# Xinglab/lr2rmats

Measured on AMD Instinct MI355X. Metric: long-read alignments classified/sec; achieved HBM GB/s vs roofline, higher is better.
Workload: dtype int32

## Files before the change

### lr2rmats_amd/csrc/l2r_engine.hip

```cpp
#include <hip/hip_runtime.h>
#include <stdarg.h>
#include <stdio.h>
#include <stdlib.h>
#include <string.h>
#include <sys/stat.h>
#include <unistd.h>
#include <algorithm>
#include <string>
#include <thread>
#include <type_traits>
#include <utility>
#include <vector>

#include "../../include/lr2rmats_hip.h"
#include "l2r_kernels.hip.h"
#include "l2r_window.hip.h"
#include "l2r_slab.hip.h"
#include "l2r_chunk.hip.h"
#include "l2r_tchunk.hip.h"
#include "l2r_filter.hip.h"
#include "l2r_fusion.hip.h"
#include "l2r_sj.hip.h"
#include "l2r_plan.hip.h"

// ... 70 lines not shown
    ~SjState() { for (int k = 0; k < 2; ++k) if (ev[k]) (void)hipEventDestroy(ev[k]); }
};
struct SjIntrons {
    DevBuf<int32_t> tx_tid, ex_start, ex_end; DevBuf<int64_t> tx_ex_off;
    SjState st;
};

struct RunFacts {
    bool known = false;
    uint32_t n_wide = 0;
    uint32_t n_chunk = 0;
    uint32_t n_rest = 0;
    uint32_t n_late = 0;
    uint32_t n_fb = 0;
    uint32_t n_wide_rest = 0;
    unsigned long long chunk_rest = 0;
    bool redo_empty = false;
};

struct l2r_ctx {
    int device = 0;
    hipStream_t stream = nullptr;
    hipStream_t side[2] = {nullptr, nullptr};
    hipEvent_t ev_fork = nullptr, ev_join[2] = {nullptr, nullptr};

    int fast_grid = 0;
    int n_cu = 256, wg_per_cu = 4;
    int ablate = 0;
    int64_t seg_max = SEG_MAX;
    Pipeline want_pipe = Pipeline::tile;
    bool pipeline_forced = false;
    bool wide_direct = true;
    bool chunk_direct = true;
    bool tile_split = true;
    bool side_on = true;
    bool env_tile_anyway = false, env_launch_all = false;
    bool check_stages = false;
    bool env_stamps = false;
    int64_t tile_resident = 0;
    bool tile_starved = false;
    int64_t n_lb_fallback = 0;

    l2r_params prm;
    std::string anno_cache_dir;
    int anno_cache_state = 0;
    unsigned want = L2R_WANT_RESULTS | L2R_WANT_ACCEPTED;
    bool one_shot_upload = false;

    bool sorted = true;
    int reads_per_tile = TILE_THREADS;
    int64_t n_tiles = 0, n_tiles256 = 0;
    bool wide_cigar = false;
    bool many_exon_reads = false;
    bool slab_ok = false;
    bool have_index = false;
    float index_ms = 0.0f;
    DevBuf<SlotRec> slot_rec;
    DevBuf<TileStat> tile_stat; std::vector<TileStat> h_tile_stat;
    DevBuf<TileStat> sup_stat;
    DevBuf<uint16_t> sum_nn;
    DevBuf<uint32_t> tile_sbase, s_pre, s_loc, s_pl, cig_off32, tile_rec, tile_total, tile_xbase, tile_span;
    DevBuf<int32_t> dense_start, dense_end;
    DevBuf<uint32_t> slab_row;
    DevBuf<TileWin> tw;
    DevBuf<TileWin64> tw64; DevBuf<uint32_t> wide_list, chunk_list, list_cnt, tile_flags;
    DevBuf<unsigned long long> ovf_cursor;
    DevBuf<unsigned long long> lb_tile, lb_blk, lb_sup;
    DevBuf<uint32_t> fb_list;
    DevBuf<uint32_t> rest_list;

    Pipeline pipe = Pipeline::classic;
    bool prev_run_tile = false;
    uint32_t lc_flip = 0;
    uint32_t lb_flip = 0;
    RunFacts facts;
    int64_t inexact_tiles = -1;
    int64_t n_tx = 0, n_anno_exon = 0;
    DevBuf<TxHdr> hdr;
    DevBuf<int2> anno_ex;
    DevBuf<int64_t> anno_key;
    DevBuf<SiteEnt> sk_st, sk_en;
    DevBuf<uint32_t> sd_st, sd_en, sr_st;
    DevBuf<int32_t> tid_base; int32_t n_tid_dir = 0;
    DevBuf<uint32_t> key_dir; DevBuf<int32_t> kb_base; int32_t n_tid_key = 0;
    DevBuf<int32_t> j0;
    int64_t n_compact = 0, n_wide = 0;
    std::vector<int64_t> h_anno_key_raw;
    std::vector<int64_t> h_anno_key_pm;
    int64_t n_sj = 0;
    DevBuf<int32_t> sj_tid, sj_don, sj_acc, sj_uniq, sj_multi;
    DevBuf<int64_t> sj_key;
    DevBuf<int32_t> sj_cbase, sj_dbase; DevBuf<uint32_t> sj_cdir, sj_ddir; DevBuf<int4> sj_row; int32_t sj_ntid = 0;
// ... 124 lines not shown
        fail(-2, "[l2r_create] hipStreamCreate: %s", hipGetErrorString(e)); delete c; return nullptr;
    }
    int prio_lo = 0, prio_hi = 0;
    (void)hipDeviceGetStreamPriorityRange(&prio_lo, &prio_hi);
    for (int k = 0; k < 2; ++k)
        if (((e = hipStreamCreateWithPriority(&c->side[k], hipStreamNonBlocking, prio_hi)) != hipSuccess &&
             ((void)hipGetLastError(), e = hipStreamCreateWithFlags(&c->side[k], hipStreamNonBlocking)) != hipSuccess) ||
            (e = hipEventCreateWithFlags(&c->ev_join[k], hipEventDisableTiming)) != hipSuccess) {
            fail(-2, "[l2r_create] side stream: %s", hipGetErrorString(e)); l2r_destroy(c); return nullptr;
        }
    if ((e = hipEventCreateWithFlags(&c->ev_fork, hipEventDisableTiming)) != hipSuccess) { fail(-2, "[l2r_create] hipEventCreate: %s", hipGetErrorString(e)); l2r_destroy(c); return nullptr; }
    c->prm = l2r_params{3, 3, 50, 0, 0x7fffffff, 5, 0, 0, 1, 0, 0.80f};
    {
        hipDeviceProp_t prop;
        if (hipGetDeviceProperties(&prop, device) == hipSuccess && prop.multiProcessorCount > 0) c->n_cu = prop.multiProcessorCount;
        const char *e = getenv("L2R_WG_PER_CU");
        if (e && atoi(e) > 0) c->wg_per_cu = atoi(e);
        e = getenv("L2R_FAST_GRID");
        if (e && atoi(e) > 0) c->fast_grid = atoi(e);
        e = getenv("L2R_ABLATE");
        c->ablate = e ? atoi(e) : 0;
        c->check_stages = getenv("L2R_CHECK") != nullptr;
        e = getenv("L2R_SEG_MAX");
        if (e && atoll(e) >= 0) c->seg_max = atoll(e);
        e = getenv("L2R_ANNO_CACHE");
        if (e && *e) c->anno_cache_dir = e;
        e = getenv("L2R_WIDE_DIRECT");
        if (e) c->wide_direct = atoi(e) != 0;
        c->env_tile_anyway = getenv("L2R_TILE_ANYWAY") != nullptr; c->env_launch_all = getenv("L2R_LAUNCH_ALL") != nullptr;
        e = getenv("L2R_CHUNK_DIRECT");
        if (e) c->chunk_direct = atoi(e) != 0;
        e = getenv("L2R_TILE_SPLIT");
        if (e) c->tile_split = atoi(e) != 0;
        e = getenv("L2R_SIDE");
        if (e) c->side_on = atoi(e) != 0;
        c->env_stamps = getenv("L2R_STAMPS") != nullptr;
        e = getenv("L2R_PIPELINE");
        if (e) { c->want_pipe = !strcmp(e, "classic") ? Pipeline::classic : !strcmp(e, "slab") ? Pipeline::slab : Pipeline::tile; c->pipeline_forced = true; }
        {
            int per_cu = 0;
            if (hipOccupancyMaxActiveBlocksPerMultiprocessor(&per_cu, k_tile<3, false, false, false>, TILE_THREADS, 0) != hipSuccess) { (void)hipGetLastError(); per_cu = 0; }
            c->tile_resident = (int64_t)per_cu * c->n_cu;
            if ((int64_t)per_cu * c->n_cu < 8 * (int64_t)TILE_GROUP + 1 || getenv("L2R_TILE_STARVED")) c->tile_starved = true;
        }
    }
    return c;
}

void l2r_destroy(l2r_ctx *c)
{
    if (!c) return;
    (void)hipSetDevice(c->device);
    for (int k = 0; k < 2; ++k) { if (c->side[k]) (void)hipStreamDestroy(c->side[k]); if (c->ev_join[k]) (void)hipEventDestroy(c->ev_join[k]); }
    if (c->ev_fork) (void)hipEventDestroy(c->ev_fork);
    if (c->stream) (void)hipStreamDestroy(c->stream);
    delete c;
}

void *l2r_stream(l2r_ctx *c) { return c ? (void *)c->stream : nullptr; }
float l2r_upload_index_ms(l2r_ctx *c) { return c ? c->index_ms : 0.0f; }
int l2r_hint_single_run(l2r_ctx *c, int on) { if (!c) return fail(-1, "[l2r_hint_single_run] null context"); c->one_shot_upload = on != 0; return 0; }

int l2r_set_outputs(l2r_ctx *c, unsigned want)
{
    if (!c) return fail(-1, "[l2r_set_outputs] null context");
    if (!(want & (L2R_WANT_RESULTS | L2R_WANT_ACCEPTED)) || (want & ~(unsigned)(L2R_WANT_RESULTS | L2R_WANT_ACCEPTED)))
// ... 492 lines not shown
    EventPair ev;
    HIP_TRY(hipEventCreate(&ev.a)); HIP_TRY(hipEventCreate(&ev.b));
    if (summaries) {
        if (c->sum_nn.ensure(N + 1)) return -2;
        HIP_TRY(hipMemcpyAsync(c->sum_nn.p, pl.nn.data(), N * 2, hipMemcpyHostToDevice, c->stream));
        HIP_TRY(hipMemcpyAsync(c->tile_stat.p, c->h_tile_stat.data(), T * sizeof(TileStat), hipMemcpyHostToDevice, c->stream));
    }
    const unsigned gi = (unsigned)std::min<size_t>(T, 8192);
    HIP_TRY(hipEventRecord(ev.a, c->stream));
    with_flag(summaries, [&](auto S) {
        hipLaunchKernelGGL(HIP_KERNEL_NAME(k_tile_index<S>), dim3(gi), dim3(TILE_THREADS), 0, c->stream, (TileRec *)c->tile_rec.p, c->tile_stat.p, c->slot_rec.p, (uint32_t)T,
                           (const uint32_t *)c->cig_off32.p, (const int32_t *)c->r_pos.p, (const uint8_t *)c->r_rev.p, (const uint32_t *)c->cig.p, S ? (const uint16_t *)c->sum_nn.p : (const uint16_t *)nullptr);
    });
    HIP_TRY(hipEventRecord(ev.b, c->stream));
    if (!summaries) {
        HIP_TRY(hipMemcpyAsync(c->h_tile_stat.data(), c->tile_stat.p, T * sizeof(TileStat), hipMemcpyDeviceToHost, c->stream));
        HIP_TRY(hipStreamSynchronize(c->stream));
    }
    HIP_TRY(hipEventSynchronize(ev.b));
    HIP_TRY(hipEventElapsedTime(&c->index_ms, ev.a, ev.b));
    return 0;
}

int l2r_upload_reads(l2r_ctx *c, const l2r_reads *r)
{
    if (!c || !r) return fail(-1, "[l2r_upload_reads] null argument");
    if (r->n_reads < 0 || r->n_cigar < 0) return fail(-1, "[l2r_upload_reads] negative size");
    if ((uint64_t)r->n_cigar + (uint64_t)r->n_reads >= 0xfffffff0ULL)
        return fail(-1, "[l2r_upload_reads] shard too large for 32-bit exon offsets (%lld ops + %lld reads); split it", (long long)r->n_cigar, (long long)r->n_reads);
    HIP_TRY(hipSetDevice(c->device));
    const int64_t N = r->n_reads;
    UploadPlan pl;
    std::vector<TileStat> sup;
    struct Drain { hipStream_t s; ~Drain() { (void)hipStreamSynchronize(s); } } drain{c->stream};
    std::string msg;
    if (int rc = plan_check_reads(*r, pl, msg)) return fail(rc, "%s", msg.c_str());

    if (int rc = stream_begin_upload(c, r)) return rc;

    PlanOpts po;
    po.min_intron = c->prm.min_intron; po.max_delet = c->prm.max_delet;
    po.want_slab = c->want_pipe != Pipeline::classic;
    po.want_index = c->want_pipe == Pipeline::tile && !(c->one_shot_upload && !c->env_tile_anyway && !c->pipeline_forced);
    po.stream_sorted = c->seq.sorted; po.last_key = c->seq.last_key;
    plan_tiles(*r, po, pl);
    c->seq.sorted = pl.sorted; c->seq.last_key = pl.last_key;
    const bool sorted = pl.sorted;
    c->sorted = sorted; c->have_win = false;
    if (!sorted || c->n_sj > 0) { c->h_tid.assign(r->tid, r->tid + N); c->h_pos.assign(r->pos, r->pos + N); }
    else { c->h_tid.clear(); c->h_pos.clear(); }
    c->wide_cigar = pl.wide_cigar; c->many_exon_reads = pl.many_exon_reads;
    c->reads_per_tile = pl.reads_per_tile; c->n_tiles = pl.n_tiles; c->n_tiles256 = pl.n_tiles256;

    if (int rc = stage_reads(c, r, pl)) return rc;
    size_t exb = 0;
    if (int rc = count_exon_bound(c, r, pl.wide_cigar, &exb)) return rc;
    if (int rc = reserve_work(c, (size_t)N, exb)) return rc;

    plan_slab(*r, exb, pl);
    c->slab_ok = pl.slab_ok; c->pipe = Pipeline::classic;
    if (pl.slab_ok) {
        if (int rc = stage_slab(c, (size_t)N, pl)) return rc;
        if (int rc = make_tile_index(c, r, pl)) return rc;
        sup = plan_sup_stat(pl, c->h_tile_stat);
        HIP_TRY(hipMemcpyAsync(c->sup_stat.p, sup.data(), sup.size() * sizeof(TileStat), hipMemcpyHostToDevice, c->stream));
    }
    if (c->env_stamps && !c->stamps.p) {
        if (c->stamps.ensure(1024 * 8 + 16)) return -2;
        HIP_TRY(hipMemsetAsync(c->stamps.p, 0, (1024 * 8 + 16) * 8, c->stream));
    }
    HIP_TRY(hipStreamSynchronize(c->stream));

    c->n_reads = N; c->n_cigar = r->n_cigar; c->first_read = r->first_read_index;
    c->ran = false; c->totals_valid = false; forget_list_state(c);
    if (sorted) {
        if (N) {
            const int64_t q = host_key(r->tid[N - 1], r->pos[N - 1] + 1);
            const int64_t at = std::upper_bound(c->h_anno_key_pm.begin(), c->h_anno_key_pm.end(), q) - c->h_anno_key_pm.begin();
            c->seq.anno_cur = std::max(c->seq.anno_cur, at);
        }
        c->seq.sj_pending = c->n_sj > 0;
    } else {
        int rc = prepare_unsorted_windows(c);
        if (rc) return rc;
    }
    return 0;
}

static int finish_stream_sj_cursor(l2r_ctx *c)
{
    l2r_ctx::Stream &st = c->seq;
    if (!st.sj_pending || !c->ran || c->n_sj == 0 || c->n_reads == 0) { st.sj_pending = false; return 0; }
    const int64_t N = c->n_reads;
    std::vector<uint32_t> info((size_t)N);
    HIP_TRY(hipMemcpyAsync(info.data(), c->info.p, (size_t)N * 4, hipMemcpyDeviceToHost, c->stream));
    HIP_TRY(hipStreamSynchronize(c->stream));
    for (int64_t i = N - 1; i >= 0; --i) {
        if ((info[(size_t)i] & (I_FULL | I_KNOWN | I_KSITE)) != (I_FULL | I_KSITE)) continue;
        const int64_t q = host_key(c->h_tid[(size_t)i], c->h_pos[(size_t)i] + 1);
// ... 85 lines not shown

static bool split_wait_free(const l2r_ctx *c) { return c->inexact_tiles == 0 && !(c->ablate & 256); }
static uint32_t split_mode(const l2r_ctx *c)
{
    if (!c->tile_split || !c->rest_list.p) return SPLIT_OFF;
    const uint32_t fits = (uint32_t)std::min<int64_t>((int64_t)c->n_cu * 4, c->tile_resident / 2);
    if (c->facts.known) return c->facts.n_rest <= fits ? SPLIT_ON : SPLIT_OFF;
    return split_wait_free(c) ? SPLIT_ON : SPLIT_LIST;
}

static SlabArgs slab_args(const l2r_ctx *c, const FastArgs &fa, const CursorDir &cd, bool tile)
{
    SlabArgs sa;
    sa.g.f = fa; sa.g.cd = cd; sa.g.tid_base = c->tid_base.p; sa.g.n_tid_dir = c->n_tid_dir; sa.g.tile_total = c->tile_total.p;
    sa.tile_sbase = c->tile_sbase.p; sa.slab_row = c->slab_row.p;
    sa.dense_start = c->dense_start.p; sa.dense_end = c->dense_end.p; sa.ovf_cursor = c->ovf_cursor.p;
    sa.pl = c->s_pl.p; sa.pre_x = c->s_pre.p; sa.loc_x = c->s_loc.p; sa.cig_off32 = c->cig_off32.p; sa.tw = c->tw.p; sa.span = (TileSpan *)c->tile_span.p;
    sa.n_tiles = (uint32_t)c->n_tiles;
    sa.tw64 = (c->ablate & 4) ? nullptr : c->tw64.p;
    sa.chunk_on = (c->ablate & 32) ? 0u : 1u;
    sa.wide_list = c->wide_list.p; sa.chunk_list = c->chunk_list.p; sa.list_cnt = c->list_cnt.p; sa.list_cnt_next = nullptr; sa.tile_flags = c->tile_flags.p;
    if (tile) { sa.list_cnt = lc_this_run(c); sa.list_cnt_next = lc_next_run(c); }
    {   const size_t sup_words = (size_t)(c->n_tiles >> LB_SUP_SHIFT) + 64;
        sa.lb_sup = c->lb_sup.p ? c->lb_sup.p + (c->lb_flip ? sup_words : 0) : nullptr;
        sa.lb_sup_next = c->lb_sup.p ? c->lb_sup.p + (c->lb_flip ? 0 : sup_words) : nullptr;
        sa.n_sup = (uint32_t)(c->n_tiles >> LB_SUP_SHIFT) + 1u; }
    sa.lb_tile = c->lb_tile.p; sa.lb_blk = c->lb_blk.p; sa.lb_err = c->totals.p + TOT_LB_ERR; sa.fb_list = c->fb_list.p; sa.exon_total = c->totals.p + TOT_EXONS; sa.tile_stat = c->tile_stat.p; sa.sup_stat = c->sup_stat.p;
    sa.sj = SjDir{CursorDir{c->sj_key.p, c->sj_cdir.p, c->sj_cbase.p, c->sj_ntid, (int32_t)c->n_sj}, c->sj_ddir.p, c->sj_dbase.p, c->sj_ntid, c->sj_row.p};
    sa.has_wide_keys = c->n_wide > 0 ? 1u : 0u;
    sa.wide_direct_on = (tile && c->wide_direct && c->tw64.p && !(c->ablate & 4)) ? 1u : 0u;
    sa.chunk_direct_on = (tile && c->chunk_direct && sa.chunk_on) ? 1u : 0u;
    sa.rest_list = c->rest_list.p;
    sa.split_on = tile ? split_mode(c) : SPLIT_OFF;
    return sa;
}

static void launch_probe(const l2r_ctx *c, const DevParams &p, const SlabArgs &sa, bool list, bool acc, unsigned grid)
{
    with_level(p.full_level, [&](auto L) { with_flag(p.ss_dis > 0, [&](auto D) { with_flag(list, [&](auto LIST) { with_flag(acc && !list, [&](auto A) {
        if constexpr (!(A && LIST))
            hipLaunchKernelGGL(HIP_KERNEL_NAME(k_probe_slab<L, A, D, LIST>), dim3(grid), dim3(TILE_THREADS), 0, c->stream, sa, (const TileSpan *)c->tile_span.p,
                               (const TileWin *)c->tw.p, (const uint32_t *)c->tile_xbase.p, (const uint32_t *)c->fb_list.p);
    }); }); }); });
}

static void launch_tile_chunk(const l2r_ctx *c, const DevParams &p, const SlabArgs &sa, unsigned grid, uint32_t late, hipStream_t s)
{
    with_level(p.full_level, [&](auto L) {
        hipLaunchKernelGGL(HIP_KERNEL_NAME(k_tile_chunk<L>), dim3(grid), dim3(TILE_THREADS), 0, s, sa, (const TileRec *)c->tile_rec.p, (const TileWin *)c->tw.p,
                           (const TileStat *)c->tile_stat.p, (const SlotRec *)c->slot_rec.p, c->tile_xbase.p, late);
    });
}

static int launch_classic(l2r_ctx *c, hipEvent_t *ev, const DevParams &p, const FastArgs &fa, const CursorDir &cd, const SiteTabs &tabs)
{
    hipStream_t s = c->stream;
    const unsigned gt = (unsigned)(c->n_tiles ? c->n_tiles : 1);
    with_flag(c->wide_cigar, [&](auto W) {
        hipLaunchKernelGGL(HIP_KERNEL_NAME(k_pass_a<W>), dim3(gt), dim3(TILE_THREADS), W ? pass_a_dynamic_lds(c->reads_per_tile) : 0, s, c->n_reads, c->r_tid.p, c->r_pos.p,
                           c->cig_off.p, c->cig.p, cd, tabs, p, (c->sorted ? (const int32_t *)nullptr : (const int32_t *)c->win_start.p), c->j0.p, c->local.p, c->order.p,
                           c->tile_base.p, c->desc.p, c->totals.p + TOT_REDO, (const TxHdr *)c->hdr.p, c->win_hdr.p, (const uint32_t *)c->tile_first.p, c->walked.p);
    });
    MARK(ST_SCAN1);
    {
        ScanJobs jobs = {}; jobs.job[0] = ScanJob{c->tile_base.p, c->n_tiles, c->totals.p + TOT_EXONS}; jobs.job[1] = jobs.job[0];
        hipLaunchKernelGGL(k_scan_u32, dim3(1), dim3(1024), 0, s, jobs);
// ... 1073 lines not shown
```

### lr2rmats_amd/csrc/l2r_plan.hip.h

```cpp
#pragma once
#include <stdarg.h>
#include <stdint.h>
#include <stdio.h>
#include <algorithm>
#include <string>
#include <vector>

#include "../../include/lr2rmats_hip.h"

namespace l2r {

struct PlanOpts {
    int32_t min_intron = 3, max_delet = 50;
    bool want_slab = true;
    bool want_index = true;
    bool stream_sorted = true;
    int64_t last_key = INT64_MIN;
};

struct UploadPlan {
    bool sorted_here = true;
    bool sorted = true;
    int64_t last_key = INT64_MIN;
    bool wide_cigar = false, many_exon_reads = false;
// ... 194 lines not shown
    pl.have_index = T && pl.make_index;
    pl.nn.clear();
    if (!pl.have_index || !r.cig_summary) return;
    pl.nn.resize((size_t)N);
    for (size_t t = 0; t < T; ++t) {
        TileStat st{0, INT32_MAX, 0, INT32_MAX};
        int64_t hi = INT32_MIN; uint32_t tot_x = 0u; bool many = false;
        for (uint32_t i = pl.tile_first[t]; i < pl.tile_first[t + 1]; ++i) {
            const uint32_t *q = r.cig_summary + 3 * (size_t)i;
            const uint32_t n_n = q[1] & 0xffffu, mn = q[1] >> 16, md = q[2] & 0xffffu, ms = q[2] >> 16;
            pl.nn[i] = (uint16_t)n_n;
            st.n_ops_n += (int32_t)n_n; st.min_n = std::min(st.min_n, (int32_t)mn); st.min_seg = std::min(st.min_seg, (int32_t)ms);
            st.max_d = std::max(st.max_d, md == 0xffffu ? INT32_MAX : (int32_t)md);
            hi = std::max<int64_t>(hi, (int64_t)r.pos[i] + (int64_t)q[0]);
            tot_x += n_n + 1u; many = many || n_n + 1u >= 255u;
        }
        if (many || tot_x >= SLOT_LOC_LIMIT) st.min_seg = INT32_MIN;
        pl.tile_stat[t] = st;
        pl.rec[t].pad[0] = (uint32_t)std::min<int64_t>(std::max<int64_t>(hi, INT32_MIN), INT32_MAX);
    }
}

static std::vector<TileStat> plan_sup_stat(const UploadPlan &pl, const std::vector<TileStat> &stat)
{
    const size_t T = (size_t)pl.n_tiles;
    std::vector<TileStat> sup((T >> LB_SUP_SHIFT) + 1, TileStat{0, INT32_MAX, 0, INT32_MAX});
    for (size_t t = 0; t < T; ++t) {
        TileStat &q = sup[t >> LB_SUP_SHIFT]; const TileStat &st = stat[t];
        q.n_ops_n += st.n_ops_n + (int32_t)pl.rec[t].n_act; q.min_n = std::min(q.min_n, st.min_n); q.max_d = std::max(q.max_d, st.max_d); q.min_seg = std::min(q.min_seg, st.min_seg);
    }
    return sup;
}

static void plan_tiles(const l2r_reads &r, const PlanOpts &o, UploadPlan &pl)
{
    plan_continuation(r, o, pl);
    plan_exon_sample(r, o, pl);
    plan_layouts(o, pl);
    plan_reads_per_tile(r, pl);
    plan_tile_cut(r, pl);
}
static void plan_slab(const l2r_reads &r, size_t exb, UploadPlan &pl)
{
    pl.slab_ok = false;
    if (!pl.slab_layout) return;
    plan_slab_layout(r, exb, pl);
    if (!pl.slab_ok) return;
    plan_tile_recs(r, pl);
    plan_summary_index(r, pl);
}

}
```

### lr2rmats_amd/csrc/l2r_slab.hip.h

```cpp
#pragma once
#include "l2r_window.hip.h"

namespace l2r {

constexpr int SLAB_ROWS = 24;
constexpr uint32_t SLAB_STRIDE = TILE_THREADS;
constexpr int SLAB_HEAD_VEC = 6;
constexpr int SLAB_HEAD = 4 * SLAB_HEAD_VEC;
constexpr int SLAB_REL_BITS = 18;
constexpr uint32_t SLAB_REL_MASK = (1u << SLAB_REL_BITS) - 1u;
constexpr uint32_t SLAB_LEN_MAX = (1u << (32 - SLAB_REL_BITS)) - 1u;
constexpr int32_t SLAB_TILE_SPAN = 1 << (SLAB_REL_BITS - 1);
__device__ __forceinline__ uint32_t slab_pack(int rel, uint32_t len) { return (uint32_t)rel | (len << SLAB_REL_BITS); }
constexpr uint32_t PRE_REV = 1u << 8;
constexpr uint32_t PRE_INSANE = 1u << 9;
constexpr uint32_t PRE_DENSE = 1u << 10;
constexpr int PRE_N_SHIFT = 11;
constexpr int PL_LOC_SHIFT = 19;
constexpr uint32_t PL_PRE_MASK = (1u << PL_LOC_SHIFT) - 1u;
constexpr uint32_t PL_N_LIMIT = 1u << (PL_LOC_SHIFT - PRE_N_SHIFT), PL_LOC_LIMIT = 1u << (32 - PL_LOC_SHIFT);

__host__ __device__ __forceinline__ uint32_t slab_rows_of(uint32_t c) { return (c + 3u) >> 1; }
__device__ __forceinline__ uint32_t slab_row(uint32_t j, uint32_t n) { return j + 1u < n ? j + 1u : 0u; }

// ... 5 lines not shown
    return st.min_n >= min_intron && st.max_d <= max_delet && st.min_seg >= min_exon;
}
constexpr int LB_SHIFT = 40;
constexpr unsigned long long LB_SUM_MASK = (1ull << LB_SHIFT) - 1ull;
constexpr int LB_BLK_SHIFT = 4, LB_BLK = 1 << LB_BLK_SHIFT, LB_SUP_SHIFT = 10;
struct SlabArgs {
    PipeArgs g;
    const uint32_t *tile_sbase;
    uint32_t *slab_row;
    int32_t *dense_start, *dense_end;
    unsigned long long *ovf_cursor;
    uint32_t *pl, *pre_x, *loc_x;
    const uint32_t *cig_off32;
    TileWin *tw;
    TileSpan *span;
    TileWin64 *tw64;
    uint32_t *wide_list, *chunk_list, *list_cnt;
    uint32_t *list_cnt_next;
    uint32_t *tile_flags;
    uint32_t chunk_on;
    uint32_t n_tiles;
    unsigned long long *lb_tile, *lb_blk, *lb_sup, *lb_sup_next;
    uint32_t n_sup;
    const TileStat *tile_stat;
    const TileStat *sup_stat;
    uint32_t *lb_err, *fb_list;
    SjDir sj;
    uint32_t has_wide_keys;
    uint32_t chunk_direct_on;
    uint32_t wide_direct_on;
    uint32_t *exon_total;
    uint32_t *rest_list;
    uint32_t split_on;
};
constexpr uint32_t SPLIT_OFF = 0u, SPLIT_ON = 1u, SPLIT_LIST = 2u;
typedef const __attribute__((address_space(4))) SlabArgs *SlabArgsK;
__device__ __forceinline__ SlabArgsK slab_args()
{
    SlabArgsK q = (SlabArgsK)__builtin_amdgcn_kernarg_segment_ptr();
    asm volatile("" : "+s"(q));
    return q;
}

__device__ __forceinline__ void chunk_list_append_late(SlabArgsK sa, uint32_t t) { sa->chunk_list[sa->n_tiles + 1u + atomicAdd(sa->list_cnt + LC_LATE, 1u)] = t; }
constexpr int SLAB_TW_VECS = (int)(sizeof(TileWin) / 16);
__device__ __forceinline__ bool tw_vec_used(int i, uint32_t n_win)
{
    if (i < WIN_TX) return (uint32_t)i < n_win;
    if (i < 2 * WIN_TX) return (uint32_t)(i - WIN_TX) < n_win;
    if (i < 2 * WIN_TX + WIN_TX / 4) return (uint32_t)(4 * (i - 2 * WIN_TX)) < n_win;
    return true;
}
__device__ __forceinline__ uint32_t xcd_tile(uint32_t b, uint32_t grid) { return (b & 7u) * (grid >> 3) + (b >> 3); }
constexpr int SLAB_KEY_CAP = 168;
static_assert(sizeof(TileWin) % 16 == 0, "TileWin is copied in 16-byte pieces");

__device__ __forceinline__ void slab_preloc(SlabArgsK sa, uint32_t t, uint32_t at, uint32_t &pre, uint32_t &loc)
{
    if (sa->span[t].fat) { pre = ld32(sa->pre_x, at); loc = ld32(sa->loc_x, at); }
    else { const uint32_t w = ld32(sa->pl, at); pre = w & PL_PRE_MASK; loc = w >> PL_LOC_SHIFT; }
}

struct WalkLds { uint32_t *cnt, *loc; int *wmax; uint32_t *wn, *nmax; };
template <bool GENERAL, bool FIRST>
__device__ __forceinline__ uint32_t slab_walk_tile(SlabArgsK sa, PipeArgsK a, uint32_t t, uint32_t r0, uint32_t n_act, uint32_t sbase, uint32_t rows_tile, int32_t tid0, int32_t pos0,
                                                   uint32_t slot, bool active, uint32_t c_lo, int32_t pos, uint32_t xw, uint32_t (&cg)[SLAB_HEAD], const WalkLds &W)
// ... 404 lines not shown
    const uint32_t t0 = (blockIdx.x - (FIRST ? 0u : n_scan)) * (uint32_t)DESCRIBE_TILES;
    const uint32_t t = t0 + (uint32_t)slot;
    uint32_t flags = TD_FAST;
    unsigned long long my_total = 0ull;
    if (FIRST && blockIdx.x == 0 && threadIdx.x == 0) {
        clear_run_counters(a->f.redo_count);
        *sa->ovf_cursor = 0ull; *sa->lb_err = 0u;
        *sa->exon_total = 0u;
        uint32_t *const lc = sa->list_cnt;
        lc[LC_WIDE_CURSOR] = 0u; lc[LC_CHUNK_CURSOR] = 0u; lc[LC_FB] = 0u; lc[LC_WIDE_REST] = 0u; lc[LC_LATE] = 0u; lc[LC_DECLINED] = 0u; lc[LC_DECLINED_LATE] = 0u;
        if (sa->list_cnt_next) { sa->list_cnt_next[LC_WIDE] = 0u; sa->list_cnt_next[LC_CHUNK] = 0u; sa->list_cnt_next[LC_REST] = 0u; }
    }
    if (FIRST && blockIdx.x == 0) for (uint32_t i = threadIdx.x; i < sa->n_sup; i += TILE_THREADS) sa->lb_sup_next[i] = 0ull;
    if (t < sa->n_tiles) {
        int4 spv, spw;
        TileStat st_first{0, 0, 0, 0}; uint32_t n_act_first = 0u;
        if (FIRST) {
            const int4 r0v = reinterpret_cast<const int4 *>(u_rec + t)[0];
            const int4 rv = reinterpret_cast<const int4 *>(u_rec + t)[1];
            const int4 sv = *reinterpret_cast<const int4 *>(sa->tile_stat + t);
            asm volatile("" :: "v"(r0v.y), "v"(rv.x), "v"(sv.x));
            st_first = TileStat{sv.x, sv.y, sv.z, sv.w}; n_act_first = (uint32_t)r0v.y;
            CursorDir cd;
            cd.key = a->cd.key; cd.dir = a->cd.dir; cd.kb_base = a->cd.kb_base; cd.n_tid = a->cd.n_tid; cd.n_tx = a->cd.n_tx;
            const int jl = cursor_value(cd, rv.x, rv.y);
            int tb = 0, nb = 0;
            if (rv.x >= 0 && rv.x < a->n_tid_dir) { tb = a->tid_base[rv.x]; nb = a->tid_base[rv.x + 1] - tb; }
            spv = make_int4(rv.x, rv.y, rv.z, 0); spw = make_int4(jl, tb, nb, 0);
            if (gl == 0) {
                const TileStat st{sv.x, sv.y, sv.z, sv.w};
                const bool exact = tile_exact(st, a->f.p.min_exon, a->f.p.min_intron, a->f.p.max_delet) && !(a->f.p.ablate & 256);
                my_total = exact ? (1ull << LB_SHIFT) | (unsigned long long)(uint32_t)(r0v.y + st.n_ops_n) : 0ull;
                sa->lb_tile[t] = my_total;
            }
        } else { spv = reinterpret_cast<const int4 *>(sa->span + t)[0]; spw = reinterpret_cast<const int4 *>(sa->span + t)[1]; }
        flags = make_descriptor<DESCRIBE_G>(a, gl, g * DESCRIBE_G, spv.x, spv.y, spv.z, sa->tw + t, sa->tw64 ? sa->tw64 + t : nullptr, s_win[slot],
                                            (uint32_t)SLAB_KEY_CAP, spw.x, spw.y, spw.z, (uint32_t)spv.w);
        if (FIRST && gl == 0 && sa->chunk_direct_on != 0u) {
            const TileDesc dd = sa->tw[t].d;
            if (tile_chunk_direct(1u, flags, sa->chunk_on, dd, st_first, n_act_first, a->f.p.min_exon, a->f.p.min_intron, a->f.p.max_delet, a->f.p.ss_dis, a->f.p.ablate)) {
                flags |= TD_CDIRECT;
                sa->tw[t].d.flags = flags;
            }
        }
        const bool xdirect = FIRST && gl == 0 && tile_exact_direct(sa->split_on, flags, sa->has_wide_keys, st_first, n_act_first, a->f.p.min_exon, a->f.p.min_intron, a->f.p.max_delet, a->f.p.ablate);
        if (xdirect && sa->split_on == SPLIT_ON) {
            flags |= TD_XDIRECT;
            sa->tw[t].d.flags = flags;
        }
        if (gl == 0) sa->tile_flags[t] = flags;
        if (xdirect) flags |= TD_XDIRECT;
        if (gl == 0 && (a->f.p.want & WANT_ACCEPTED)) a->f.tile_chunk[t] = CHUNK_DEFERRED;
    }
    if (gl == 0) s_flags[slot] = flags;
    if (FIRST && gl == 0) { s_tot[slot][0] = (uint32_t)my_total; s_tot[slot][1] = (uint32_t)(my_total >> 32); }
    __syncthreads();
    if (FIRST && wv == 1 && t0 < sa->n_tiles) {
        const uint32_t lo = lane < DESCRIBE_TILES ? s_tot[lane][0] : 0u, hi = lane < DESCRIBE_TILES ? s_tot[lane][1] : 0u;
        const unsigned long long sum = ((unsigned long long)wave_sum(hi) << 32) + (unsigned long long)wave_sum(lo);
        if (lane == 0) {
            sa->lb_blk[t0 >> LB_BLK_SHIFT] = sum;
            const int4 qv = *reinterpret_cast<const int4 *>(sa->sup_stat + (t0 >> LB_SUP_SHIFT));
            const TileStat q{qv.x, qv.y, qv.z, qv.w};
            const bool whole = tile_exact(q, a->f.p.min_exon, a->f.p.min_intron, a->f.p.max_delet) && !(a->f.p.ablate & 256) &&
                               ((t0 >> LB_SUP_SHIFT) + 1u) << LB_SUP_SHIFT <= sa->n_tiles;
            const uint32_t in_blk = min((uint32_t)LB_BLK, sa->n_tiles - t0);
// ... 472 lines not shown
```

### lr2rmats_amd/csrc/l2r_tile.hip.h

```cpp
#pragma once
#include <type_traits>
#include "l2r_chunk.hip.h"

namespace l2r {

#ifndef L2R_TILE_GROUP_SHIFT
#define L2R_TILE_GROUP_SHIFT 4
#endif
constexpr uint32_t TILE_GROUP = 1u << L2R_TILE_GROUP_SHIFT;
#ifndef L2R_TILE_EXACT_WALK
#define L2R_TILE_EXACT_WALK 1
#endif
__device__ __forceinline__ uint32_t fused_tile(uint32_t b)
{
    const uint32_t x = b & 7u, i = b >> 3;
    return ((((i >> L2R_TILE_GROUP_SHIFT) << 3) + x) << L2R_TILE_GROUP_SHIFT) + (i & (TILE_GROUP - 1u));
}
inline unsigned fused_grid(int64_t n_tiles)
{
    const int64_t per = 8 * (int64_t)TILE_GROUP;
    return (unsigned)(std::max<int64_t>((n_tiles + per - 1) / per, 1) * per);
}

struct SlotRec { uint32_t c_lo; int32_t pos; uint32_t xw; };
// ... 423 lines not shown
    constexpr int DIR_BYTES = FAST_DIR_BYTES;
    using WinT = typename std::conditional<WIDE, TileWin64, TileWin>::type;
    using EntT = typename std::conditional<WIDE, WEnt, v4i_t>::type;
    constexpr int AUX_BYTES = SLAB_DIR_BYTES + (int)sizeof(WinT);
    static_assert(AUX_BYTES >= SLAB_AUX_BYTES && WIDE_KEY_CAP == SLAB_KEY_CAP, "the WIDE instance's arrays hold what the plain one's do");
    __shared__ __attribute__((aligned(16))) uint32_t s_A[TILE_POS_CAP];
    __shared__ __attribute__((aligned(16))) uint16_t s_L[TILE_POS_CAP];
    __shared__ __attribute__((aligned(16))) EntT s_ent[2 * SLAB_KEY_CAP];
    __shared__ __attribute__((aligned(16))) uint8_t s_aux[AUX_BYTES];
    __shared__ __attribute__((aligned(16))) uint8_t s_cnt[TILE_THREADS];
    __shared__ __attribute__((aligned(16))) uint16_t s_loc[TILE_THREADS];
    __shared__ uint32_t s_flagw[TILE_THREADS / WAVE], s_redow[TILE_THREADS / WAVE];
    __shared__ uint32_t s_lb[4];
    __shared__ uint32_t s_chunk[2];
    uint8_t *const s_dir = s_aux;
    WinT &s_tw = *reinterpret_cast<WinT *>(s_aux + SLAB_DIR_BYTES);
    (void)kernarg_block;
    const SlabArgsK sa = slab_args();
    const PipeArgsK a = pipe_args();
    const int lane = threadIdx.x & (WAVE - 1), wv = threadIdx.x >> 6;
    uint32_t t;
    if (WIDE) { if (blockIdx.x >= sa->list_cnt[LC_WIDE]) return; t = sa->wide_list[blockIdx.x]; }
    else if (!EXACT && sa->split_on == SPLIT_ON) { if (blockIdx.x >= sa->list_cnt[LC_REST]) return; t = sa->rest_list[blockIdx.x]; }
    else { t = fused_tile(blockIdx.x); if (t >= sa->n_tiles) return; }
    SlabStamp stamp; stamp.start(a->f.stamps); if (stamp.who == 3) stamp.who = -1;
    __builtin_amdgcn_s_setprio(TILE_PRIO);
    const uint32_t clk0 = stamp.p ? (uint32_t)__builtin_amdgcn_s_memrealtime() : 0u;
    const v3u_a4 srec = *reinterpret_cast<const v3u_a4 *>(u_slot + ((size_t)t * TILE_THREADS + threadIdx.x));
    const TileRec rec = u_rec[t];
    const TileDesc d0 = WIDE ? sa->tw64[t].d : u_tw[t].d;
    const TileStat tst = u_stat[t];
    const uint32_t chunk_on = sa->chunk_on; const int32_t ablate = a->f.p.ablate;
    const uint32_t n_tiles = sa->n_tiles;
    if constexpr (EXACT)
        asm volatile("" :: "s"(tst.n_ops_n), "s"(ablate), "s"(n_tiles), "s"(rec.r0), "s"(rec.n_act), "s"(rec.tid0), "s"(rec.lo),
                           "s"(d0.j_lo), "s"(d0.b_off), "s"(d0.nb), "s"(d0.b0), "s"(d0.nbk), "s"(d0.st_r0), "s"(d0.st_nk), "s"(d0.en_r0), "s"(d0.en_nk), "s"(d0.flags), "s"(d0.n_win));
    else
    asm volatile("" :: "s"(tst.n_ops_n), "s"(tst.min_n), "s"(tst.max_d), "s"(tst.min_seg), "s"(chunk_on), "s"(ablate), "s"(n_tiles), "s"(rec.r0), "s"(rec.n_act), "s"(rec.sbase), "s"(rec.rows), "s"(rec.tid0), "s"(rec.lo),
                       "s"(d0.j_lo), "s"(d0.b_off), "s"(d0.nb), "s"(d0.b0), "s"(d0.nbk), "s"(d0.st_r0), "s"(d0.st_nk), "s"(d0.en_r0), "s"(d0.en_nk), "s"(d0.flags), "s"(d0.n_win));
    if (EXACT && (d0.flags & TD_XDIRECT) == 0u) return;
    const uint32_t r0 = rec.r0, n_act = rec.n_act;
    const int32_t tid0 = rec.tid0, pos0 = rec.lo - 1;
    const int32_t tile_lo = rec.lo;
    const bool pre_slab = !WIDE && !EXACT && ((d0.flags & TD_WIDE) != 0u || (chunk_on && slab_tile_is_chunked(d0.flags)));
    const bool counted = EXACT || (tile_exact(tst, a->f.p.min_exon, a->f.p.min_intron, a->f.p.max_delet) && !(ablate & 256));
    if constexpr (!EXACT) {
        const bool direct = tile_wide_direct(sa->wide_direct_on, d0.flags, chunk_on, tst, n_act, a->f.p.min_exon, a->f.p.min_intron, a->f.p.max_delet, ablate);
        if (WIDE ? !direct : direct) return;
        if (!WIDE && (d0.flags & TD_CDIRECT) != 0u) return;
    }
    TileDesc d = d0;
    if (pre_slab) d.flags = 0u;
    EntT *const s_ent0 = s_ent, *const s_ent1 = s_ent + SLAB_KEY_CAP;
    uint8_t *const s_dir0 = s_dir, *const s_dir1 = s_dir + DIR_BYTES, *const s_rdir = s_dir + 2 * DIR_BYTES;
    LbLevel lv{nullptr, 0u, 0u};
    unsigned long long ev = 0ull;
    if (wv < 3 && !pre_slab) { lv = lb_level(sa, t, wv); if ((uint32_t)lane < lv.cnt) ev = lv.p[lane]; }
    const DictRegs dv = load_dict_slices(a, d);
    int4 twv = make_int4(0, 0, 0, 0);
    if (WIDE) { if ((int)threadIdx.x < WIDE_TW_VECS) twv = reinterpret_cast<const int4 *>(sa->tw64 + t)[threadIdx.x]; }
    else if ((int)threadIdx.x < SLAB_TW_VECS && tw_vec_used((int)threadIdx.x, (d.flags & TD_FAST) ? d.n_win : 0u)) twv = reinterpret_cast<const int4 *>(u_tw + t)[threadIdx.x];
    const uint32_t c_lo = srec.x, xs = srec.z;
    const int32_t pos = (int32_t)srec.y;
    const bool active = (xs & SLOT_VALID) != 0u;
    const uint32_t n_cig = xs & 0xffu, idx = (xs >> SLOT_IDX_SHIFT) & 0xffu;
    uint32_t cg[SLAB_HEAD];
#pragma unroll
    for (int i = 0; i < SLAB_HEAD; ++i) cg[i] = 1u;
    if (active) {
        const uint32_t *const words = a->f.cig + c_lo;
#pragma unroll
        for (int q = 0; q < SLAB_HEAD_VEC; ++q)
            if ((uint32_t)(4 * q) < n_cig) {
                const v4i_a4 x = *reinterpret_cast<const v4i_a4 *>(words + 4 * q);
                cg[4 * q] = (uint32_t)x.x; cg[4 * q + 1] = (uint32_t)x.y; cg[4 * q + 2] = (uint32_t)x.z; cg[4 * q + 3] = (uint32_t)x.w;
            }
    }
    bool first_look = false;
    uint32_t first_share = 0u;
    if (wv < 3 && !pre_slab) {
        const bool in = (uint32_t)lane < lv.cnt;
        first_look = __all(!in || (uint32_t)(ev >> LB_SHIFT) == lv.want) && lv.cnt <= (uint32_t)WAVE;
        first_share = wave_sum(in ? (uint32_t)ev : 0u);
    }
    if (!pre_slab && (int)threadIdx.x < (WIDE ? WIDE_TW_VECS : SLAB_TW_VECS)) reinterpret_cast<int4 *>(&s_tw)[threadIdx.x] = twv;
    int my_wide = 0;
    if constexpr (WIDE) wide_stage_dict(d, dv, reinterpret_cast<const int *>(sa->tw64[t].win), s_ent0, s_ent1, s_dir0, s_dir1, s_rdir);
    else if (EXACT) (void)slab_stage_dict(d, dv, reinterpret_cast<const int *>(u_tw[t].win), SlabLds{nullptr, s_ent0, s_ent1, s_dir0, s_dir1, s_rdir});
    else if (!pre_slab) my_wide = slab_stage_dict(d, dv, reinterpret_cast<const int *>(u_tw[t].win), SlabLds{nullptr, s_ent0, s_ent1, s_dir0, s_dir1, s_rdir});
    stamp.mark(0);
#pragma unroll
    for (int i = 0; i < SLAB_HEAD; ++i) if ((i & 3) || WIDE) cg[i] = (uint32_t)i < n_cig ? cg[i] : 1u;
    DevParams p;
    p.min_exon = a->f.p.min_exon; p.min_intron = a->f.p.min_intron; p.max_delet = a->f.p.max_delet;
    const uint32_t t3 = ((uint32_t)p.min_intron << 4) | 3u, t2 = ((uint32_t)(p.max_delet + 1) << 4) | 2u;
    const int c_max = wave_max(active ? (int)min(n_cig, (uint32_t)SLAB_HEAD) : 0);
    uint32_t n = 0u;
    const bool meet = !WIDE && !EXACT && !pre_slab && (!counted || sa->has_wide_keys != 0u);
    if constexpr (!EXACT) {
    if (!pre_slab && !counted) {
        if (active) {
            int start = pos + 1, end = pos;
            bool first = true;
            auto step = [&](uint32_t c) {
                const uint32_t op = c & 0xfu;
                const int len = (int)(c >> 4);
                const bool cut = ((op == 3u) & (c >= t3)) | ((op == 2u) & (c >= t2));
                const bool keep = cut & (first | (end - start >= p.min_exon - 1));
                n += keep ? 1u : 0u;
                first = first & !keep;
                start = cut ? end + len + 1 : start;
                end += len & __builtin_amdgcn_sbfe(0x18d, op, 1u);
            };
// ... 15 lines not shown
        __syncthreads();
    }
    }
    stamp.mark(1);
    uint32_t total = 0u, loc = 0u;
    bool late_slab = false, wide_key = false;
    int any_wide = 0;
    if constexpr (EXACT) { total = n_act + (uint32_t)tst.n_ops_n; loc = (xs >> SLOT_LOC_SHIFT) & (SLOT_LOC_LIMIT - 1u); }
    else if (!pre_slab) {
        if (counted) { total = n_act + (uint32_t)tst.n_ops_n; loc = (xs >> SLOT_LOC_SHIFT) & (SLOT_LOC_LIMIT - 1u); }
        else {
            const uint32_t c4 = reinterpret_cast<const uint32_t *>(s_cnt)[lane];
            const uint32_t b0 = c4 & 0xffu, b1 = (c4 >> 8) & 0xffu, b2 = (c4 >> 16) & 0xffu, b3 = c4 >> 24;
            const uint32_t sum = b0 + b1 + b2 + b3;
            const uint32_t inc = wave_inclusive_scan(sum), ex = inc - sum;
            reinterpret_cast<uint2 *>(s_loc)[lane] = make_uint2(ex | ((ex + b0) << 16), (ex + b0 + b1) | ((ex + b0 + b1 + b2) << 16));
            total = (uint32_t)__builtin_amdgcn_readlane((int)inc, WAVE - 1);
            loc = s_loc[idx];
        }
        const uint32_t fl = meet ? (uint32_t)__builtin_amdgcn_readfirstlane((int)(s_flagw[0] | s_flagw[1] | s_flagw[2] | s_flagw[3])) : 0u;
        late_slab = total > (uint32_t)TILE_POS_CAP || (fl & 1u) != 0u || ((fl & 2u) != 0u && chunk_on != 0u);
        wide_key = (fl & 2u) != 0u;
        any_wide = (wide_key && !late_slab) ? 1 : 0;
    }
    auto staged_form = [&]() {
    if constexpr (!EXACT) if (threadIdx.x == 0 && !counted && !(ablate & 128) && !((ablate & 32768) && t == 3u)) lb_publish(sa, t, total);
    const uint32_t clk1 = stamp.p ? (uint32_t)__builtin_amdgcn_s_memrealtime() : 0u;
    const SlabStage st{s_A, s_L, loc, tile_lo, true};
    ReadEnds re{0, 0, 0, 0};
    bool sane = true, big = false;
    n = 0u;
    if (active && (EXACT || (L2R_TILE_EXACT_WALK && counted))) {
        uint32_t *const Ap = s_A + loc;
        uint32_t *wp = Ap;
        uint32_t rel = (uint32_t)(pos + 1 - tile_lo), xl = 0u, longest = 0u;
        auto step = [&](uint32_t c) {
            const uint32_t op = c & 0xfu, len = c >> 4;
            const bool is_n = op == 3u;
            if (is_n) *wp = slab_pack((int)rel, xl);
            wp += is_n ? 1 : 0;
            longest = max(longest, xl);
            rel += is_n ? xl + len : 0u;
            xl = is_n ? 0u : xl + (len & (uint32_t)__builtin_amdgcn_sbfe(0x18d, op, 1u));
        };
#pragma unroll
        for (int q = 0; q < SLAB_HEAD_VEC; ++q)
            if (4 * q < c_max) { step(cg[4 * q]); step(cg[4 * q + 1]); step(cg[4 * q + 2]); step(cg[4 * q + 3]); }
        if (n_cig > (uint32_t)SLAB_HEAD) {
            const uint32_t n_ops = ld32(sa->cig_off32, r0 + idx + 1u) - c_lo;
            const uint32_t *const words = a->f.cig + c_lo;
            for (uint32_t i = SLAB_HEAD; i < n_ops; ++i) step(words[i]);
        }
        *wp = slab_pack((int)rel, xl);
        longest = max(longest, xl);
        if (rel >= SLAB_REL_MASK) longest = 0xffffffffu;
        n = (uint32_t)(wp - Ap) + 1u;
        big = longest > SLAB_LEN_MAX;
        const uint32_t x0 = Ap[0] >> SLAB_REL_BITS;
        sane = x0 >= 1u && xl >= 1u;
        const int start = tile_lo + (int)rel;
        re = ReadEnds{pos + 1, pos + (int)x0, start, start + (int)xl - 1};
    } else if constexpr (!EXACT) if (active) {
        uint32_t *const Ap = s_A + loc;
        int start = pos + 1, end = pos;
        int s0 = 0, e0 = 0;
        bool first = true;
        uint32_t longest = 0u;
        auto step = [&](uint32_t c) {
            const uint32_t op = c & 0xfu;
            const int len = (int)(c >> 4);
            const bool cut = ((op == 3u) & (c >= t3)) | ((op == 2u) & (c >= t2));
            const bool keep = cut & (first | (end - start >= p.min_exon - 1));
            if (keep) {
                const uint32_t xlen = (uint32_t)(end - start + 1);
                Ap[n] = slab_pack(start - tile_lo, xlen);
                longest = max(longest, xlen);
                if (first) { s0 = start; e0 = end; }
                first = false; ++n;
            }
            start = cut ? end + len + 1 : start;
            end += len & __builtin_amdgcn_sbfe(0x18d, op, 1u);
        };
#pragma unroll
        for (int q = 0; q < SLAB_HEAD_VEC; ++q)
            if (4 * q < c_max) { step(cg[4 * q]); step(cg[4 * q + 1]); step(cg[4 * q + 2]); step(cg[4 * q + 3]); }
        if (n_cig > (uint32_t)SLAB_HEAD) {
            const uint32_t n_ops = ld32(sa->cig_off32, r0 + idx + 1u) - c_lo;
            const uint32_t *const words = a->f.cig + c_lo;
            for (uint32_t i = SLAB_HEAD; i < n_ops; ++i) step(words[i]);
        }
// ... 97 lines not shown
                const int r_start = tile_lo + (int)(s_A[loc] & SLAB_REL_MASK);
                const int r_end = tile_lo + (int)(s_A[loc + n - 1u] & SLAB_REL_MASK) + (int)s_L[loc + n - 1u] - 1;
                from = cursor_value(sd.cur, tid0, r_start);
                if (from < n_sj) ok0 = !(from >= ti0.end || sd.row[from].x >= r_end);
            }
            s_sjfrom[threadIdx.x] = (cand && ok0) ? from : -1;
            s_bad[threadIdx.x] = 0;
            if (active) for (uint32_t k = 0; k < n; ++k) s_owner[loc + k] = (uint8_t)threadIdx.x;
            __syncthreads();
            for (uint32_t q = threadIdx.x; q < total; q += (uint32_t)TILE_THREADS) {
                const uint32_t av = s_A[q];
                if (av == SLAB_POS_SKIP || !((av >> SLAB_REL_BITS) & F_JUNC)) continue;
                const uint32_t who = s_owner[q];
                const int fr = s_sjfrom[who];
                if (fr < 0) continue;
                const int don = tile_lo + (int)(av & SLAB_REL_MASK) + (int)s_L[q], acc = tile_lo + (int)(s_A[q + 1u] & SLAB_REL_MASK) - 1;
                if (!junction_supported(ti0, don, acc, fr, pj, sd)) { s_A[q] = av | ((uint32_t)F_UNREL << SLAB_REL_BITS); s_bad[who] = 1; }
            }
            __syncthreads();
            if (cand) {
                const bool ok = ok0 && s_bad[threadIdx.x] == 0;
                vd.info |= I_SJCHK | (ok ? I_SJPASS : I_UNREL);
                if (ok || a->f.p.split_trans) vd.info |= I_ACCEPT;
            }
        }
    }
    if (active) a->f.info[r] = vd.info;
    uint32_t clk2 = 0u;
    {
        uint32_t share = first_share;
        uint32_t n_polls = 0u;
        bool done;
        clk2 = stamp.p ? (uint32_t)__builtin_amdgcn_s_memrealtime() : 0u;
        if (wv < 3 && !first_look && !(ablate & 64)) share = lb_share<false>(sa, t, wv, lane, done, n_polls);
        if (stamp.p && lane == 0 && wv < 3) { atomicAdd(&stamp.p[8192 + wv], (unsigned long long)n_polls); atomicAdd(&stamp.p[8192 + 3 + wv], n_polls ? 1ull : 0ull); }
        if (ablate & 64) share = wv == 0 ? t * (uint32_t)TILE_POS_CAP : 0u;
        if (lane == 0 && wv < 3) s_lb[wv] = share;
    }
    __syncthreads();
    if (stamp.p && threadIdx.x == 0) {
        uint32_t xcc;
        asm volatile("s_getreg_b32 %0, hwreg(HW_REG_XCC_ID)" : "=s"(xcc));
        a->tile_total[t] = (clk0 << 3) | (xcc & 7u); a->f.tile_acc[t] = clk1; a->f.tile_acc_ex[t] = clk2;
        sa->tile_flags[t] = (uint32_t)__builtin_amdgcn_s_memrealtime();
    }
    stamp.mark(7);
    const uint32_t xbase = (uint32_t)__builtin_amdgcn_readfirstlane((int)(s_lb[0] + s_lb[1] + s_lb[2]));
    if (threadIdx.x == 0) {
        u_xbase[t] = xbase;
        if (t + 1u == n_tiles) { u_xbase[n_tiles] = xbase + total; *sa->exon_total = xbase + total; }
    }
    const SlabOut out{a->f.ex_start, a->f.ex_end, a->f.ex_flag, xbase + loc};
    if (active) a->f.ex_off[r] = out.dst;
    if (active && big) {
        const uint32_t n_ops = ld32(sa->cig_off32, r + 1u) - c_lo;
        const uint32_t *const words = a->f.cig + c_lo;
        WalkState w{pos + 1, pos, 0};
        auto put = [&](int k, int s_, int e_) { out.start[out.dst + (uint32_t)k] = s_; out.end[out.dst + (uint32_t)k] = e_; out.flag[out.dst + (uint32_t)k] = 0; };
        walk_ops<false>(w, words, 0, (int)n_ops, p, put);
        put(w.n, w.start, w.end);
    }
    if (!ACC) {
        slab_write_out(SlabOut{out.start, out.end, out.flag, xbase}, s_A, s_L, tile_lo, total);
        stamp.mark(5);
        return;
    }
    const bool fused = __builtin_amdgcn_readfirstlane((int)(s_redow[0] | s_redow[1] | s_redow[2] | s_redow[3])) == 0 && !(ablate & 2);
    if (!fused) { slab_write_out(SlabOut{out.start, out.end, out.flag, xbase}, s_A, s_L, tile_lo, total); return; }
    uint32_t *const s_racc = reinterpret_cast<uint32_t *>(s_aux), *const s_rscan = s_racc + TILE_THREADS;
    uint16_t *const s_map = reinterpret_cast<uint16_t *>(s_ent);
    const bool acc = active && (vd.info & I_ACCEPT) != 0u;
    s_racc[idx] = acc ? ((1u << 16) | n) : 0u;
    __syncthreads();
    uint32_t ca, cx;
    {
        const uint4 c4 = reinterpret_cast<const uint4 *>(s_racc)[lane];
        const uint32_t sum = c4.x + c4.y + c4.z + c4.w;
        const uint32_t inc = wave_inclusive_scan(sum), ex = inc - sum;
        reinterpret_cast<uint4 *>(s_rscan)[lane] = make_uint4(ex, ex + c4.x, ex + c4.x + c4.y, ex + c4.x + c4.y + c4.z);
        const uint32_t tot = (uint32_t)__builtin_amdgcn_readlane((int)inc, WAVE - 1);
        ca = tot >> 16; cx = tot & 0xffffu;
    }
// ... 95 lines not shown
```

Before: 22.27 billion.

## Precompute per-tile exon offsets on host to skip decoupled lookback

For exact tiles, the host now computes a prefix sum of per-tile exon counts during upload and stores it on the device. The describe stage writes each tile's base offset, so the tile kernel reads it from a scalar load instead of polling the lookback chain. This removes inter-tile serialization and spin-waiting. The exact-walk inner loop is also rewritten to be branch-free, with unconditional LDS stores, bitfield extracts and inline asm pointer advance. The cost is a host-side scan and an extra upload, plus reliance on exact host-side counts.

```diff
diff --git a/lr2rmats_amd/csrc/l2r_engine.hip b/lr2rmats_amd/csrc/l2r_engine.hip
--- a/lr2rmats_amd/csrc/l2r_engine.hip
+++ b/lr2rmats_amd/csrc/l2r_engine.hip
@@ -126,6 +126,7 @@
     bool pipeline_forced = false;
     bool wide_direct = true;
     bool chunk_direct = true;
+    bool xfront_on = true;
     bool tile_split = true;
     bool side_on = true;
     bool env_tile_anyway = false, env_launch_all = false;
@@ -152,6 +153,8 @@
     DevBuf<SlotRec> slot_rec;
     DevBuf<TileStat> tile_stat; std::vector<TileStat> h_tile_stat;
     DevBuf<TileStat> sup_stat;
+    DevBuf<uint32_t> tile_xfront;
+    bool have_xfront = false;
     DevBuf<uint16_t> sum_nn;
     DevBuf<uint32_t> tile_sbase, s_pre, s_loc, s_pl, cig_off32, tile_rec, tile_total, tile_xbase, tile_span;
     DevBuf<int32_t> dense_start, dense_end;
@@ -342,6 +345,8 @@
         if (e) c->chunk_direct = atoi(e) != 0;
         e = getenv("L2R_TILE_SPLIT");
         if (e) c->tile_split = atoi(e) != 0;
+        e = getenv("L2R_XFRONT");
+        if (e) c->xfront_on = atoi(e) != 0;
         e = getenv("L2R_SIDE");
         if (e) c->side_on = atoi(e) != 0;
         c->env_stamps = getenv("L2R_STAMPS") != nullptr;
@@ -900,6 +905,7 @@
     const int64_t N = r->n_reads;
     UploadPlan pl;
     std::vector<TileStat> sup;
+    std::vector<uint32_t> front;
     struct Drain { hipStream_t s; ~Drain() { (void)hipStreamSynchronize(s); } } drain{c->stream};
     std::string msg;
     if (int rc = plan_check_reads(*r, pl, msg)) return fail(rc, "%s", msg.c_str());
@@ -932,7 +938,13 @@
         if (int rc = make_tile_index(c, r, pl)) return rc;
         sup = plan_sup_stat(pl, c->h_tile_stat);
         HIP_TRY(hipMemcpyAsync(c->sup_stat.p, sup.data(), sup.size() * sizeof(TileStat), hipMemcpyHostToDevice, c->stream));
-    }
+        c->have_xfront = c->have_index && c->h_tile_stat.size() == (size_t)pl.n_tiles && pl.rec.size() >= (size_t)pl.n_tiles;
+        if (c->have_xfront) {
+            front = plan_exon_front(pl, c->h_tile_stat);
+            if (c->tile_xfront.ensure(front.size())) return -2;
+            HIP_TRY(hipMemcpyAsync(c->tile_xfront.p, front.data(), front.size() * 4, hipMemcpyHostToDevice, c->stream));
+        }
+    } else c->have_xfront = false;
     if (c->env_stamps && !c->stamps.p) {
         if (c->stamps.ensure(1024 * 8 + 16)) return -2;
         HIP_TRY(hipMemsetAsync(c->stamps.p, 0, (1024 * 8 + 16) * 8, c->stream));
@@ -1084,6 +1096,7 @@
     sa.chunk_direct_on = (tile && c->chunk_direct && sa.chunk_on) ? 1u : 0u;
     sa.rest_list = c->rest_list.p;
     sa.split_on = tile ? split_mode(c) : SPLIT_OFF;
+    sa.xfront = (tile && c->have_xfront && c->xfront_on && split_wait_free(c)) ? (const uint32_t *)c->tile_xfront.p : nullptr;
     return sa;
 }
 
diff --git a/lr2rmats_amd/csrc/l2r_plan.hip.h b/lr2rmats_amd/csrc/l2r_plan.hip.h
--- a/lr2rmats_amd/csrc/l2r_plan.hip.h
+++ b/lr2rmats_amd/csrc/l2r_plan.hip.h
@@ -250,6 +250,14 @@
     return sup;
 }
 
+static std::vector<uint32_t> plan_exon_front(const UploadPlan &pl, const std::vector<TileStat> &stat)
+{
+    const size_t T = (size_t)pl.n_tiles;
+    std::vector<uint32_t> front(T + 1, 0u);
+    for (size_t t = 0; t < T; ++t) front[t + 1] = front[t] + pl.rec[t].n_act + (uint32_t)stat[t].n_ops_n;
+    return front;
+}
+
 static void plan_tiles(const l2r_reads &r, const PlanOpts &o, UploadPlan &pl)
 {
     plan_continuation(r, o, pl);
diff --git a/lr2rmats_amd/csrc/l2r_slab.hip.h b/lr2rmats_amd/csrc/l2r_slab.hip.h
--- a/lr2rmats_amd/csrc/l2r_slab.hip.h
+++ b/lr2rmats_amd/csrc/l2r_slab.hip.h
@@ -61,6 +61,7 @@
     uint32_t *exon_total;
     uint32_t *rest_list;
     uint32_t split_on;
+    const uint32_t *xfront;
 };
 constexpr uint32_t SPLIT_OFF = 0u, SPLIT_ON = 1u, SPLIT_LIST = 2u;
 typedef const __attribute__((address_space(4))) SlabArgs *SlabArgsK;
@@ -531,6 +532,7 @@
                 const bool exact = tile_exact(st, a->f.p.min_exon, a->f.p.min_intron, a->f.p.max_delet) && !(a->f.p.ablate & 256);
                 my_total = exact ? (1ull << LB_SHIFT) | (unsigned long long)(uint32_t)(r0v.y + st.n_ops_n) : 0ull;
                 sa->lb_tile[t] = my_total;
+                if (sa->xfront) job.out[t] = sa->xfront[t];
             }
         } else { spv = reinterpret_cast<const int4 *>(sa->span + t)[0]; spw = reinterpret_cast<const int4 *>(sa->span + t)[1]; }
         flags = make_descriptor<DESCRIBE_G>(a, gl, g * DESCRIBE_G, spv.x, spv.y, spv.z, sa->tw + t, sa->tw64 ? sa->tw64 + t : nullptr, s_win[slot],
diff --git a/lr2rmats_amd/csrc/l2r_tile.hip.h b/lr2rmats_amd/csrc/l2r_tile.hip.h
--- a/lr2rmats_amd/csrc/l2r_tile.hip.h
+++ b/lr2rmats_amd/csrc/l2r_tile.hip.h
@@ -479,8 +479,10 @@
     const TileStat tst = u_stat[t];
     const uint32_t chunk_on = sa->chunk_on; const int32_t ablate = a->f.p.ablate;
     const uint32_t n_tiles = sa->n_tiles;
+    const bool scanned = EXACT && sa->xfront != nullptr;
+    const uint32_t xb_scan = EXACT ? *(const __attribute__((address_space(4))) uint32_t *)(u_xbase + t) : 0u;
     if constexpr (EXACT)
-        asm volatile("" :: "s"(tst.n_ops_n), "s"(ablate), "s"(n_tiles), "s"(rec.r0), "s"(rec.n_act), "s"(rec.tid0), "s"(rec.lo),
+        asm volatile("" :: "s"(tst.n_ops_n), "s"(ablate), "s"(n_tiles), "s"(xb_scan), "s"(rec.r0), "s"(rec.n_act), "s"(rec.tid0), "s"(rec.lo),
                            "s"(d0.j_lo), "s"(d0.b_off), "s"(d0.nb), "s"(d0.b0), "s"(d0.nbk), "s"(d0.st_r0), "s"(d0.st_nk), "s"(d0.en_r0), "s"(d0.en_nk), "s"(d0.flags), "s"(d0.n_win));
     else
     asm volatile("" :: "s"(tst.n_ops_n), "s"(tst.min_n), "s"(tst.max_d), "s"(tst.min_seg), "s"(chunk_on), "s"(ablate), "s"(n_tiles), "s"(rec.r0), "s"(rec.n_act), "s"(rec.sbase), "s"(rec.rows), "s"(rec.tid0), "s"(rec.lo),
@@ -502,7 +504,7 @@
     uint8_t *const s_dir0 = s_dir, *const s_dir1 = s_dir + DIR_BYTES, *const s_rdir = s_dir + 2 * DIR_BYTES;
     LbLevel lv{nullptr, 0u, 0u};
     unsigned long long ev = 0ull;
-    if (wv < 3 && !pre_slab) { lv = lb_level(sa, t, wv); if ((uint32_t)lane < lv.cnt) ev = lv.p[lane]; }
+    if (wv < 3 && !pre_slab && !scanned) { lv = lb_level(sa, t, wv); if ((uint32_t)lane < lv.cnt) ev = lv.p[lane]; }
     const DictRegs dv = load_dict_slices(a, d);
     int4 twv = make_int4(0, 0, 0, 0);
     if (WIDE) { if ((int)threadIdx.x < WIDE_TW_VECS) twv = reinterpret_cast<const int4 *>(sa->tw64 + t)[threadIdx.x]; }
@@ -525,7 +527,7 @@
     }
     bool first_look = false;
     uint32_t first_share = 0u;
-    if (wv < 3 && !pre_slab) {
+    if (wv < 3 && !pre_slab && !scanned) {
         const bool in = (uint32_t)lane < lv.cnt;
         first_look = __all(!in || (uint32_t)(ev >> LB_SHIFT) == lv.want) && lv.cnt <= (uint32_t)WAVE;
         first_share = wave_sum(in ? (uint32_t)ev : 0u);
@@ -607,16 +609,20 @@
     n = 0u;
     if (active && (EXACT || (L2R_TILE_EXACT_WALK && counted))) {
         uint32_t *const Ap = s_A + loc;
-        uint32_t *wp = Ap;
-        uint32_t rel = (uint32_t)(pos + 1 - tile_lo), xl = 0u, longest = 0u;
+        typedef __attribute__((address_space(3))) uint32_t lds_u32;
+        const uint32_t wp0 = (uint32_t)(uintptr_t)(lds_u32 *)Ap;
+        uint32_t wp = wp0;
+        uint32_t rel = (uint32_t)(pos + 1 - tile_lo), e = rel, over = 0u;
         auto step = [&](uint32_t c) {
-            const uint32_t op = c & 0xfu, len = c >> 4;
-            const bool is_n = op == 3u;
-            if (is_n) *wp = slab_pack((int)rel, xl);
-            wp += is_n ? 1 : 0;
-            longest = max(longest, xl);
-            rel += is_n ? xl + len : 0u;
-            xl = is_n ? 0u : xl + (len & (uint32_t)__builtin_amdgcn_sbfe(0x18d, op, 1u));
+            const uint32_t is_n = (uint32_t)__builtin_amdgcn_sbfe(0x00080008, c, 1u);
+            const uint32_t adv = (uint32_t)__builtin_amdgcn_sbfe(0x018d018d, c, 1u);
+            const uint32_t xl = e - rel;
+            *(lds_u32 *)(uintptr_t)wp = slab_pack((int)rel, xl);
+            over |= xl;
+            e += (c >> 4) & adv;
+            asm("v_mad_i32_i24 %0, %1, -4, %0" : "+v"(wp) : "v"(is_n));
+            rel = (e & is_n) | (rel & ~is_n);
+            asm volatile("" : "+v"(rel));
         };
 #pragma unroll
         for (int q = 0; q < SLAB_HEAD_VEC; ++q)
@@ -626,11 +632,11 @@
             const uint32_t *const words = a->f.cig + c_lo;
             for (uint32_t i = SLAB_HEAD; i < n_ops; ++i) step(words[i]);
         }
-        *wp = slab_pack((int)rel, xl);
-        longest = max(longest, xl);
-        if (rel >= SLAB_REL_MASK) longest = 0xffffffffu;
-        n = (uint32_t)(wp - Ap) + 1u;
-        big = longest > SLAB_LEN_MAX;
+        const uint32_t xl = e - rel;
+        *(lds_u32 *)(uintptr_t)wp = slab_pack((int)rel, xl);
+        over |= xl;
+        n = ((wp - wp0) >> 2) + 1u;
+        big = over > SLAB_LEN_MAX || rel >= SLAB_REL_MASK;
         const uint32_t x0 = Ap[0] >> SLAB_REL_BITS;
         sane = x0 >= 1u && xl >= 1u;
         const int start = tile_lo + (int)rel;
@@ -794,7 +800,7 @@
         uint32_t n_polls = 0u;
         bool done;
         clk2 = stamp.p ? (uint32_t)__builtin_amdgcn_s_memrealtime() : 0u;
-        if (wv < 3 && !first_look && !(ablate & 64)) share = lb_share<false>(sa, t, wv, lane, done, n_polls);
+        if (wv < 3 && !first_look && !(ablate & 64) && !scanned) share = lb_share<false>(sa, t, wv, lane, done, n_polls);
         if (stamp.p && lane == 0 && wv < 3) { atomicAdd(&stamp.p[8192 + wv], (unsigned long long)n_polls); atomicAdd(&stamp.p[8192 + 3 + wv], n_polls ? 1ull : 0ull); }
         if (ablate & 64) share = wv == 0 ? t * (uint32_t)TILE_POS_CAP : 0u;
         if (lane == 0 && wv < 3) s_lb[wv] = share;
@@ -807,9 +813,9 @@
         sa->tile_flags[t] = (uint32_t)__builtin_amdgcn_s_memrealtime();
     }
     stamp.mark(7);
-    const uint32_t xbase = (uint32_t)__builtin_amdgcn_readfirstlane((int)(s_lb[0] + s_lb[1] + s_lb[2]));
+    const uint32_t xbase = (scanned && !(ablate & 64)) ? xb_scan : (uint32_t)__builtin_amdgcn_readfirstlane((int)(s_lb[0] + s_lb[1] + s_lb[2]));
     if (threadIdx.x == 0) {
-        u_xbase[t] = xbase;
+        if (!scanned) u_xbase[t] = xbase;
         if (t + 1u == n_tiles) { u_xbase[n_tiles] = xbase + total; *sa->exon_total = xbase + total; }
     }
     const SlabOut out{a->f.ex_start, a->f.ex_end, a->f.ex_flag, xbase + loc};
```

Measured after the change: 22.52 billion, median of 5. 1.01x the previous value.
